# facebookresearch/dietgpu

Hardware: AMD Instinct MI355X
Metric: rans_encode_decode_GBps (higher is better)
Workload: dtype u8 (byte-wise rANS on the split exponent plane of 16-bit words); 1 GPU; 256x524288 bfloat16 N(0,1), float codec, probBits 10 (BASELINE config 3); per_gpu_batch_bytes=268435456, api=C ABI: dgpu_float_compress + dgpu_float_decompress

## Files before the change

dietgpu_amd/_lib.py:

```python
import ctypes as C
import os

from .build import LIB_PATH

_lib = None

u32, i32, sz, vp = C.c_uint32, C.c_int, C.c_size_t, C.c_void_p
_SIGS = {
    "dgpu_version": (C.c_char_p, []),
    "dgpu_abi_version": (u32, []),
    "dgpu_last_error": (C.c_char_p, []),
    "dgpu_last_checksum_mismatches": (C.c_uint32, [C.POINTER(C.c_int32), C.POINTER(C.c_uint32), C.POINTER(C.c_uint32), C.c_uint32]),
    "dgpu_ans_max_compressed_size": (u32, [u32]),
    "dgpu_float_max_compressed_size": (u32, [u32, u32]),
    "dgpu_ans_encode_temp_bytes": (sz, [u32, u32]),
    "dgpu_ans_decode_temp_bytes": (sz, [u32, u32, i32]),
    "dgpu_float_compress_temp_bytes": (sz, [u32, u32, u32]),
    "dgpu_float_decompress_temp_bytes": (sz, [u32, u32, u32, i32]),
    "dgpu_ans_encode_batch_stride": (i32, [vp, sz, vp, i32, i32, u32, vp, u32, u32, vp, vp, u32, vp, vp]),
    "dgpu_ans_encode_batch_pointer": (i32, [vp, sz, vp, i32, i32, u32, vp, vp, vp, vp, vp, vp]),
    "dgpu_ans_encode_batch_split_size": (i32, [vp, sz, vp, i32, i32, u32, vp, vp, vp, vp, u32, vp, vp]),
    "dgpu_ans_decode_batch_stride": (i32, [vp, sz, vp, i32, i32, u32, vp, u32, vp, u32, u32, vp, vp, vp, vp]),
    "dgpu_ans_decode_batch_pointer": (i32, [vp, sz, vp, i32, i32, u32, vp, vp, vp, vp, vp, vp, vp]),
    "dgpu_ans_decode_batch_split_size": (i32, [vp, sz, vp, i32, i32, u32, vp, vp, vp, vp, vp, vp, vp]),
# ... 25 lines not shown
    "dgpu_float_reduce_compress_scaled": (i32, [vp, sz, vp, u32, i32, i32, u32, u32, vp, vp, vp, C.c_float, vp, vp, vp, vp, vp, vp, vp]),
    "dgpu_float_reduce_norm_temp_bytes": (sz, [u32, u32, u32, i32]),
    "dgpu_float_decode_reduce_norm": (i32, [vp, sz, vp, u32, i32, i32, u32, u32, vp, vp, vp, C.c_float, vp, vp, vp, vp, vp, vp, vp]),
    "dgpu_float_reduce_compress_norm": (i32, [vp, sz, vp, u32, i32, i32, u32, u32, vp, vp, vp, C.c_float, vp, vp, vp, vp, vp, vp, vp, vp, vp]),
    "dgpu_float_compress_stride_capped": (i32, [vp, sz, vp, u32, i32, i32, u32, vp, u32, u32, vp, u32, u32, vp, vp]),
    "dgpu_float_decompress_stride_bounded": (i32, [vp, sz, vp, u32, i32, i32, u32, vp, u32, u32, vp, u32, u32, vp, vp, vp, vp]),
    "dgpu_float_get_compressed_info": (i32, [vp, sz, vp, u32, vp, vp, vp, vp]),
    "dgpu_float_get_compressed_info_device": (i32, [vp, u32, vp, vp, vp, vp]),
    "dgpu_ans_histogram_batch_stride": (i32, [u32, vp, u32, u32, vp, vp]),
    "dgpu_ans_calc_weights": (i32, [u32, i32, vp, u32, vp, vp, vp]),
    "dgpu_release_stream_state": (i32, [vp]),
    "dgpu_release_all_stream_state": (i32, []),
    "dgpu_debug_stream_state_count": (u32, []),
    "dgpu_debug_counters_nonzero": (C.c_int64, [vp]),
    "dgpu_prof_enable": (None, [i32]),
    "dgpu_prof_reset": (None, []),
    "dgpu_prof_summary": (i32, [C.c_char_p, sz]),
    "dgpu_debug_set_absent_workgroups": (None, [u32]),
    "dgpu_debug_set_encoder_dispatch": (None, [i32]),
    "dgpu_debug_set_decoder_order": (None, [i32]),
    "dgpu_debug_set_param_cache": (None, [i32]),
    "dgpu_debug_set_work_lists": (None, [i32]),
    "dgpu_debug_set_size_classes": (None, [i32]),
    "dgpu_set_histogram_load_policy": (None, [i32]),
    "dgpu_release_graph_state": (i32, []),
}

EXPORTED_SYMBOLS = tuple(_SIGS)


def lib():
    global _lib
    if _lib is None:
        if not os.path.exists(LIB_PATH):
            raise ImportError(
                f"{LIB_PATH} is missing: the HIP extension has not been built "
                "(run `python -m dietgpu_amd.build`). There is no CPU fallback."
            )
        L = C.CDLL(LIB_PATH)
        for name, (res, args) in _SIGS.items():
            if os.environ.get("DGPU_LIB") and not hasattr(L, name):
                continue
            fn = getattr(L, name)
            fn.restype = res
            fn.argtypes = args
        _lib = L
# ... 12 lines not shown
```

dietgpu_amd/build.py:

```python
import os
import subprocess

_HERE = os.path.dirname(os.path.abspath(__file__))
CSRC = os.path.join(_HERE, "csrc")
LIB_DIR = os.path.join(_HERE, "lib")
LIB_PATH = os.environ.get("DGPU_LIB") or os.path.join(LIB_DIR, "libdietgpu_amd.so")

_SOURCES = ["capi.hip"]


def _deps():
    names = sorted(f for f in os.listdir(CSRC) if f.endswith((".h", ".hip")))
    return [os.path.join(CSRC, f) for f in names] + [os.path.join(_HERE, "..", "include", "dietgpu_amd.h")]


def needs_build():
    if not os.path.exists(LIB_PATH):
        return True
    t = os.path.getmtime(LIB_PATH)
    return any(os.path.getmtime(d) > t for d in _deps())


def build(force=False, verbose=False):
    if not force and not needs_build():
        return LIB_PATH
    os.makedirs(LIB_DIR, exist_ok=True)
    cmd = ["hipcc", "--offload-arch=gfx950", "-O3", "-std=c++17", "-fPIC", "-shared",
           "-o", LIB_PATH] + [os.path.join(CSRC, s) for s in _SOURCES]
    if verbose:
        print(" ".join(cmd))
    subprocess.check_call(cmd)
    return LIB_PATH


TORCH_LIB_PATH = os.path.join(LIB_DIR, "libdietgpu_torch.so")


def build_torch_ops(force=False, verbose=False):
    src = os.path.join(CSRC, "torch_ops.cpp")
    if (not force and os.path.exists(TORCH_LIB_PATH)
            and os.path.getmtime(TORCH_LIB_PATH) >= max(os.path.getmtime(src), os.path.getmtime(LIB_PATH))):
        return TORCH_LIB_PATH
    import torch

    tl = os.path.dirname(torch.__file__)
    abi = int(torch._C._GLIBCXX_USE_CXX11_ABI)
    cmd = ["g++", "-O2", "-std=c++17", "-fPIC", "-shared", "-D__HIP_PLATFORM_AMD__", "-DUSE_ROCM",
           f"-D_GLIBCXX_USE_CXX11_ABI={abi}", f"-I{tl}/include", f"-I{tl}/include/torch/csrc/api/include",
           "-I/opt/rocm/include", src, "-o", TORCH_LIB_PATH, f"-L{LIB_DIR}", "-ldietgpu_amd", f"-L{tl}/lib",
           "-ltorch", "-ltorch_cpu", "-lc10", "-lc10_hip", "-ltorch_hip", "-Wl,-rpath,$ORIGIN"]
    if verbose:
        print(" ".join(cmd))
    subprocess.check_call(cmd)
    return TORCH_LIB_PATH
# ... 6 lines not shown
```

dietgpu_amd/csrc/capi.hip:

```cpp
#include "../../include/dietgpu_amd.h"

#include <hip/hip_runtime.h>

#include <algorithm>
#include <atomic>
#include <climits>
#include <cmath>
#include <cstdio>
#include <cstdlib>
#include <cstring>
#include <map>
#include <mutex>
#include <string>
#include <thread>
#include <vector>

#include "format.h"
#include "kernel_variants.h"
#include "work_plan.h"

using namespace dgpu;

namespace {

// ... 1071 lines not shown
  if (done) return rc;
  return encodeBatch(temp_dev, tempBytes, tempUsed, 0u, P, useChecksum, b, histogram_dev, outSize_dev, stream);
}

int floatCompressImpl(
    void* temp_dev, size_t tempBytes, size_t* tempUsed, uint32_t ft, int P, int useChecksum, Batch& b, uint32_t* outSize_dev,
    hipStream_t stream, bool cast = false, const RollingCounts& rolling = RollingCounts{}, bool feedback = false) {
  bool done;
  int rc = checkCall(P, b.n, ft, tempUsed,  nullptr, &done,
                     "tensor larger than 1717538816 words: the maximum compressed size of its exponent plane exceeds INT32_MAX (GpuANSEncode.cu:22)",
                     b.maxSize);
  if (done) return rc;
  const uint32_t source = feedback ? (ft | kCastSource | kFeedbackSource) : (cast ? (ft | kCastSource) : ft);
  return encodeBatch(temp_dev, tempBytes, tempUsed, source, P, useChecksum, b, nullptr, outSize_dev, stream, 0xffffffffu, rolling);
}

std::atomic<int> g_decOrder{envInt("DGPU_DEC_ORDER", -1)};
uint32_t decodeOrder(uint32_t B) {
  const int forced = g_decOrder.load();
  if (forced >= 0 && forced <= (int)kDecOrderXcd) return (uint32_t)forced;
  return B >= 64u ? kDecOrderXcd : kDecOrderElementMajor;
}

DecodeArgs decodeArgs(const Batch& b, const DeviceBatch& d, uint32_t ft, uint8_t* outSuccess_dev, uint32_t* outSize_dev) {
  DecodeArgs a;
  a.in = d.in;
  a.out = d.out;
  a.floatType = ft;
  a.outSuccess = outSuccess_dev;
  a.outSize = outSize_dev;
  a.inBytes = d.inBytes;
  a.uniformInBytes = b.uniformInBytes;
  a.numInBatch = b.n;
  return a;
}

int launchDecode(DecodeArgs d, const LaunchGroup& g, const uint32_t* work_dev, DecodeForm form, int P, hipStream_t stream) {
  const bool pairs = g.tileBlocks == kDecBlocksPerSingleTile;
  const uint32_t B = d.numInBatch;
  d.maxTiles = g.maxTiles;
  d.order = g.listed ? kDecOrderMap : decodeOrder(B);
  d.workMap = g.listed ? work_dev + (pairs ? g.elemsAt : g.tilesAt) : nullptr;
  d.numListed = g.numElems;
  const uint32_t tiles = g.listed ? std::max(g.numTiles, 1u) : (d.order == kDecOrderXcd ? roundUp(B, 8u) : B) * g.maxTiles;
  const uint32_t grid = pairs ? ((g.listed ? g.numElems : B) + 1u) / 2u : tiles;
  return launchVariant(decoderVariant(P, d.floatType, g.tileBlocks, form), dim3(grid), stream, d);
}

int decodeImpl(
    void* temp_dev, size_t tempBytes, size_t* tempUsed, uint32_t ft, int P, int useChecksum, Batch& b, uint8_t* outSuccess_dev,
    uint32_t* outSize_dev, hipStream_t stream, int32_t* errBatch) {
  g_mismatches.clear();
  bool done;
  int rc = checkCall(P, b.n, ft, tempUsed, errBatch, &done);
  if (done) return rc;
  const uint32_t B = b.n, maxCapacity = b.maxSize;
  StreamLease streamLease(stream);
  if (useChecksum && streamLease.capturing()) {
    return fail(DGPU_ERR_HIP, "HIP graph capture: checksum verification on decode copies to the host and synchronises the "
                              "stream; it cannot be captured into a HIP graph (decode with useChecksum = 0 under capture)");
  }

  TempArena arena(temp_dev, tempBytes, streamLease);
  DeviceBatch dev;
  std::vector<LaunchGroup> groups{decodeRectangle(divUp(maxCapacity, kBlockSize), true)};
  rc = resolveBatch(b, true, streamLease, &dev, [&] { planDecodeCall(planPolicy(), b.sizes, maxCapacity, true, &groups, &b.work); });
  if (rc) return rc;

  uint32_t* sizesForChecksum = outSize_dev;
// ... 392 lines not shown

uint32_t dgpu_last_checksum_mismatches(int32_t* batchIdx, uint32_t* expected, uint32_t* got, uint32_t cap) {
  const uint32_t n = (uint32_t)g_mismatches.size();
  for (uint32_t i = 0; i < n && i < cap; ++i) {
    if (batchIdx) batchIdx[i] = g_mismatches[i].batch;
    if (expected) expected[i] = g_mismatches[i].expected;
    if (got) got[i] = g_mismatches[i].got;
  }
  return n;
}

static std::atomic<uint32_t> g_absentModulo{0};
}
namespace {
uint32_t absentWorkgroupModulo() { return g_absentModulo.load(); }
}
extern "C" {
void dgpu_debug_set_absent_workgroups(uint32_t modulo) { g_absentModulo.store(modulo); }
void dgpu_debug_set_encoder_dispatch(int mode) { g_encDispatch.store(mode < 0 ? -1 : (mode != 0)); }
void dgpu_debug_set_decoder_order(int order) { g_decOrder.store(order); }
void dgpu_debug_set_param_cache(int on) { g_paramCacheEnabled.store(on != 0); }
void dgpu_debug_set_work_lists(int mode) { g_workLists.store(mode < 0 ? -1 : (mode ? 1 : 0)); }
void dgpu_debug_set_size_classes(int mode) { g_sizeClasses.store(mode < 0 ? -1 : (mode ? 1 : 0)); }
void dgpu_set_histogram_load_policy(int mode) { g_histLoadPolicy.store(mode < 0 ? -1 : (mode != 0)); }
int dgpu_release_graph_state(void) {
  const int n = paramCache().releaseGraphPins();
  return n + streamRegistry().release(nullptr, true, true);
}

int dgpu_release_stream_state(void* stream) { return streamRegistry().release((hipStream_t)stream, false); }
int dgpu_release_all_stream_state(void) { return streamRegistry().release(nullptr, true); }
uint32_t dgpu_debug_stream_state_count(void) { return (uint32_t)streamRegistry().size(); }
int64_t dgpu_debug_counters_nonzero(void* stream) {
  hipStreamCaptureStatus st = hipStreamCaptureStatusNone;
  if (hipStreamIsCapturing((hipStream_t)stream, &st) != hipSuccess || st != hipStreamCaptureStatusNone) {
    (void)hipGetLastError();
    return -1;
  }
  hipError_t e = hipSuccess;
  StreamState* s = streamRegistry().acquire((hipStream_t)stream, &e, false);
  if (!s) return -1;
  int64_t n = -1;
  std::vector<uint32_t> host(kCounterWordsArrive + kCounterWordsAcc + kCounterWordsSpill);
  if (s->counters && hipStreamSynchronize((hipStream_t)stream) == hipSuccess &&
      hipMemcpy(host.data(), s->counters, host.size() * sizeof(uint32_t), hipMemcpyDeviceToHost) == hipSuccess) {
    n = (int64_t)std::count_if(host.begin(), host.end(), [](uint32_t w) { return w != 0u; });
// ... 646 lines not shown
```

dietgpu_amd/csrc/kernel_variants.h:

```cpp
#pragma once

#include <hip/hip_runtime.h>

#include <map>
#include <mutex>
#include <type_traits>

#include "format.h"
#include "kernels_decode.h"
#include "kernels_encode.h"
#include "kernels_pairs.h"
#include "kernels_stats.h"

namespace dgpu {

template <typename... Args>
struct KernelVariant {
  void (*fn)(Args...);
  uint32_t threads;
  uint32_t ldsBytes;
  const char* name;
};
using EncodeVariant = KernelVariant<EncodeArgs>;
using DecodeVariant = KernelVariant<DecodeArgs>;
using HistogramVariant = KernelVariant<BatchView, uint32_t*, uint32_t, HistFuse>;
using StatsSingleVariant = KernelVariant<BatchView, NormalizeArgs, const uint32_t*, uint32_t>;

template <typename... Args>
uint32_t workgroupsPerCu(const KernelVariant<Args...>& v) {
  static std::mutex mu;
  static std::map<const void*, uint32_t> cache;
// ... 104 lines not shown
    return tiled(UintC<kBlocksPerTile>{}, yes, no);
  });
}

constexpr uint32_t sameType(uint32_t ft) { return ft; }
constexpr uint32_t floatsOnly(uint32_t ft) { return ft ? ft : kFloat32; }
constexpr uint32_t halvesOnly(uint32_t ft) { return ft == kFloat16 ? kFloat16 : kBFloat16; }

#define DGPU_DECODE_FORMS(X)                                                                                           \
  X(kAccum, k_ans_decode_accum, floatsOnly, decLdsBytes(P, T, TB))                                                     \
  X(kReduce, k_ans_decode_reduce, floatsOnly, decLdsBytes(P, T, TB))                                                   \
  X(kReduceStats, k_ans_decode_reduce_stats, halvesOnly, decReduceStatsLdsBytes(P, T, TB))                             \
  X(kReduceMixed, k_ans_decode_reduce_mixed, floatsOnly, decLdsBytes(P, T, TB))                                        \
  X(kReduceMixedStats, k_ans_decode_reduce_mixed_stats, halvesOnly, decReduceStatsLdsBytes(P, T, TB))                  \
  X(kReduceScaled, k_ans_decode_reduce_mixed_scaled, floatsOnly, decLdsBytes(P, T, TB))                                \
  X(kReduceScaledStats, k_ans_decode_reduce_mixed_stats_scaled, halvesOnly, decReduceStatsScaledLdsBytes(P, T, TB))    \
  X(kReduceNorm, k_ans_decode_reduce_mixed_norm, floatsOnly, decReduceNormLdsBytes(P, T, TB, false))                   \
  X(kReduceNormStats, k_ans_decode_reduce_mixed_stats_norm, halvesOnly, decReduceNormLdsBytes(P, T, TB, true))         \
  X(kWholeScaled, k_ans_decode_scaled, floatsOnly, decScaledLdsBytes(P, T, TB))                                        \
  X(kAccumScaled, k_ans_decode_accum_scaled, floatsOnly, decLdsBytes(P, T, TB))                                        \
  X(kUpdate, k_ans_decode_update, halvesOnly, decLdsBytes(P, T, TB))                                                   \
  X(kRanged, k_ans_decode_range, sameType, decLdsBytes(P, T, TB))

inline DecodeVariant decoderVariant(int P, uint32_t ft, uint32_t tileBlocks, DecodeForm form = DecodeForm::kWhole) {
  return withProbBitsAndFloatType(P, ft, [&](auto p, auto f) -> DecodeVariant {
    constexpr int kP = decltype(p)::value;
    constexpr uint32_t kFT = decltype(f)::value;
    auto smallOrFull = [&](auto tiled) -> DecodeVariant {
      return tileBlocks <= kDecBlocksPerSmallTile ? tiled(UintC<kDecBlocksPerSmallTile>{}) : tiled(UintC<kDecBlocksPerTile>{});
    };
#define DGPU_DECODE_FORM_CASE(formName, kernel, typeOf, ldsBytes)                \
  if (form == DecodeForm::formName) {                                            \
    return smallOrFull([](auto tb) -> DecodeVariant {                            \
      constexpr int P = kP;                                                      \
      constexpr uint32_t T = typeOf(kFT), TB = decltype(tb)::value;              \
      return {kernel<P, T, TB>, decThreads(TB), ldsBytes, #kernel};              \
    });                                                                          \
  }
    DGPU_DECODE_FORMS(DGPU_DECODE_FORM_CASE)
#undef DGPU_DECODE_FORM_CASE
    if (tileBlocks == kDecBlocksPerSingleTile) return {k_ans_decode_pair<kP, kFT>, 64u, decPairLdsBytes(kP, kFT), "k_ans_decode_pair"};
    auto tiled = [](auto tb) -> DecodeVariant {
      constexpr uint32_t kTB = decltype(tb)::value;
      return {k_ans_decode<kP, kFT, kTB>, decThreads(kTB), decLdsBytes(kP, kFT, kTB), "k_ans_decode"};
    };
    if (tileBlocks == kDecBlocksPerTinyTile) return tiled(UintC<kDecBlocksPerTinyTile>{});
    if (tileBlocks == kDecBlocksPerSmallTile) return tiled(UintC<kDecBlocksPerSmallTile>{});
    return tiled(UintC<kDecBlocksPerTile>{});
  });
}

inline HistogramVariant histogramVariant(uint32_t ft, bool smallBins, bool nonTemporal) {
  auto pick = [&](auto f) -> HistogramVariant {
    constexpr uint32_t kFT = decltype(f)::value;
    auto of = [](auto slots, auto nt) -> HistogramVariant {
      constexpr uint32_t kS = decltype(slots)::value;
      constexpr bool kNt = decltype(nt)::value;
      if constexpr (kFT == 0) {
        return {k_histogram<kS, kNt>, 256u, 0u, "k_histogram"};
      } else {
        return {k_float_histogram<kFT, kS, kNt>, 256u, 0u,
                encIsFeedback(kFT) ? "k_float_histogram_feedback" : (encIsCast(kFT) ? "k_float_histogram_cast" : "k_float_histogram")};
      }
    };
    constexpr UintC<kHistSlotsSmall> small{};
    constexpr UintC<kHistSlotsLarge> large{};
// ... 20 lines not shown
```

dietgpu_amd/csrc/kernels_decode.h:

```cpp
#pragma once
#include <type_traits>

#include "format.h"
#include "plan_constants.h"
#include "kernels_stats.h"

namespace dgpu {

__device__ __forceinline__ const uint8_t* locateAns(const uint8_t* archive, uint32_t ft, uint32_t* floatSize) {
  if (!ft) return archive;
  const FloatHeader fh = *(const FloatHeader*)archive;
  if (floatSize) *floatSize = fh.size;
  return archive + 16u + floatUncompDataSize(ft, fh.size);
}

struct DecodeArgs {
  BatchView in;
  BatchView out;
  uint32_t floatType;
  uint8_t* outSuccess;
  uint32_t* outSize;
  const uint32_t* inBytes;
  uint32_t numInBatch;
  uint32_t maxTiles;
// ... 592 lines not shown
struct DecodePreOf {
  uint4 words[4];
  GroupPre nc[2];
};
typedef DecodePreOf<uint2> DecodePre;
template <uint32_t FT, typename Sink>
__device__ __forceinline__ void decodePrefetch(DecodePreOf<typename Sink::GroupPre>& pre, const uint8_t* __restrict__ gwords, uint32_t numWords,
                                               const Sink& sink, uint32_t hl, bool wide) {
  const uint32_t paddedBytes = roundUp(numWords, kBlockAlignWords) * 2u;
#pragma unroll
  for (uint32_t k = 0; k < 4u; ++k) {
    const uint32_t off = (k * 32u + hl) * 16u;
    pre.words[k] = make_uint4(0, 0, 0, 0);
    if (off < paddedBytes) pre.words[k] = decLoad16(gwords + off);
  }
  pre.nc[0] = pre.nc[1] = typename Sink::GroupPre();
  if (wide) {
    pre.nc[0] = sink.prefetchGroup(kRowsPerBlock / 8u - 1u, hl);
    pre.nc[1] = sink.prefetchGroup(kRowsPerBlock / 8u - 2u, hl);
  }
}

template <int P, uint32_t FT, bool kFull, bool kWide = false, bool kIdleUpper = false, bool kCompact = false, bool kNoRing = false,
          bool kPre = false, bool kTail = false, typename Sink = RowSink<FT>>
__device__ __forceinline__ void decodeBlock(
    uint32_t xpose,
    uint32_t state,
    uint32_t n,
    uint32_t groups,
    const uint8_t* __restrict__ gwords,
    uint32_t numWords,
    uint32_t ringBase,
    const void* __restrict__ lutRaw,
    const Sink& sink,
    uint32_t hl,
    bool upper,
    const DecodePreOf<typename Sink::GroupPre>* pre = nullptr,
    uint32_t topRows = 0) {
  static_assert(!kPre || (kNoRing && kFull), "");
  static_assert(!kTail || (kFull && !kPre), "");
  constexpr uint32_t kMask = (1u << P) - 1u;
  const uint32_t laneMaskLt = (1u << hl) - 1u;
  auto lutAt = [&](uint32_t x) -> uint2 {
    if (kCompact) {
      const uint32_t e = ((const uint32_t*)lutRaw)[x];
      return make_uint2((e & 0xff000fffu), (e >> 12) & 0xfffu);
    }
// ... 57 lines not shown
  int upperSel = (upper && !kIdleUpper) ? 1 : 0;
  asm volatile("" : "+v"(upperSel));
  auto stepFull = [&]() -> uint32_t {
    const uint2 e = lutAt(state & kMask);
    state = __umul24(e.x, state >> P) + e.y;
    const bool read = state < kMinState;
    const uint64_t vote = __ballot(read);
    const uint32_t vLo = (uint32_t)vote, vHi = (uint32_t)(vote >> 32);
    const uint32_t sLoOld = sLo;
    sLo -= (uint32_t)__popc(vLo);
    sHi -= (uint32_t)__popc(vHi);
    uint32_t t = __builtin_amdgcn_mbcnt_hi(vHi, __builtin_amdgcn_mbcnt_lo(vLo, 0u));
    t = (uint32_t)(__mul24(upperSel, (int)(sHi - sLoOld)) + (int)t);
    asm volatile("" : "+v"(t));
    const uint32_t addr = kNoRing ? ((t + sLo) << 1) : ((((t + sLo) << 1) & (kRingBytes - 1u)) | ringBase);
    const uint32_t w = *(const LdsU16*)(uintptr_t)addr;
    state = read ? ((state << kEncodedBits) | w) : state;
    return e.x;
  };

  auto runGroups = [&](auto fullTag, const int gHi, const int gLo) {
    constexpr bool F = decltype(fullTag)::value;
    constexpr bool kJoinAtFlush = F && kWide;
    Pre preCur[kGroupRows], preNext[kGroupRows];
    GroupPre ncCur = GroupPre(), ncNext = GroupPre(), ncNext2 = GroupPre();
    if (kJoinAtFlush) {
      if (kPre) {
        ncCur = pre->nc[0];
        ncNext = pre->nc[1];
      } else {
        ncCur = sink.prefetchGroup((uint32_t)gHi, hl);
        ncNext = sink.prefetchGroup(gHi > gLo ? (uint32_t)(gHi - 1) : (uint32_t)gLo, hl);
      }
    }
#pragma unroll
    for (int j = 0; j < (int)kGroupRows; ++j) {
      const uint32_t row = (uint32_t)gHi * kGroupRows + j;
      preCur[j] = kJoinAtFlush ? (Pre)0 : ((F || row * 32u + hl < n) ? sink.prefetch(row) : (Pre)0);
    }

#pragma unroll 1
    for (int g = gHi; g >= gLo; --g) {
      const uint32_t gNext = g > gLo ? (uint32_t)(g - 1) : (uint32_t)gLo;
      if (kJoinAtFlush) {
        ncNext2 = sink.prefetchGroup(g > gLo + 1 ? (uint32_t)(g - 2) : (uint32_t)gLo, hl);
      } else {
// ... 39 lines not shown
      } else {
#pragma unroll
        for (int j = 0; j < (int)kGroupRows; ++j) preCur[j] = preNext[j];
      }
    }
  };

  if (kTail) {
    if (topRows != 0u) runGroups(std::false_type{}, (int)(groups + divUp(topRows, kGroupRows)) - 1, (int)groups);
    if (groups == 0u) return;
  }
  if (kFull) {
    sLo = __builtin_amdgcn_readlane(posw, 0);
    sHi = __builtin_amdgcn_readlane(posw, 32);
    if (kNoRing) {
      sLo += __builtin_amdgcn_readlane(ringBase, 0) >> 1;
      sHi += __builtin_amdgcn_readlane(ringBase, 32) >> 1;
    }
  }
  runGroups(std::integral_constant<bool, kFull>{}, (int)groups - 1, 0);
}

enum class DecodeForm { kWhole, kRanged, kAccum, kReduce, kReduceStats, kReduceMixed, kReduceMixedStats, kReduceScaled, kReduceScaledStats, kReduceNorm, kReduceNormStats, kWholeScaled, kAccumScaled, kUpdate };
template <int P, uint32_t FT, uint32_t kTileBlocks, DecodeForm kForm>
__device__ __forceinline__ void decodeTile(const DecodeArgs& a) {
  constexpr bool kRanged = kForm == DecodeForm::kRanged, kAccumScaled = kForm == DecodeForm::kAccumScaled;
  constexpr bool kUpdate = kForm == DecodeForm::kUpdate;
  constexpr bool kAccum = kForm == DecodeForm::kAccum || kAccumScaled || kUpdate;
  constexpr bool kScaledForm = kForm == DecodeForm::kWholeScaled || kAccumScaled || kUpdate;
  static_assert(kForm == DecodeForm::kWhole || kForm == DecodeForm::kRanged || kAccum || kScaledForm,
                "decode-reduce has a body of its own: decodeReduceTile");
  static_assert(!(kAccum || kScaledForm) || FT != 0u, "accumulating and scaled decode: float archives only");
  static_assert(!kUpdate || FT == kFloat16 || FT == kBFloat16, "decode-update: 16-bit float archives only");
  using Sink = std::conditional_t<kUpdate, UpdateSink<kUpdate ? FT : kBFloat16>,
                                  std::conditional_t<kAccum, AccumSink<FT ? FT : kFloat32, 0u, false, false, kAccumScaled>,
                                                     std::conditional_t<kScaledForm, ScaledSink<FT ? FT : kFloat32>, RowSink<FT>>>>;
  constexpr uint32_t kDecThreads = decThreads(kTileBlocks);
  static_assert(kTileBlocks * kRingBytes >= 2048u, "");
  extern __shared__ __attribute__((aligned(16))) uint8_t smem[];
  uint2* sLut = (uint2*)(smem + kTileBlocks * kRingBytes);
  constexpr uint32_t kXpose = decXposeBytes(P, FT, kTileBlocks);

  const uint32_t tid = threadIdx.x;
  const uint32_t lane = tid & 63u;
  const uint32_t wave = tid >> 6;
  const bool upper = lane >= 32u;
  const uint32_t hl = lane & 31u;
  const uint32_t hw = wave * 2u + (upper ? 1u : 0u);
// ... 241 lines not shown
        carry = dmax(carry, (uint32_t)__builtin_amdgcn_readlane((int)incl, 63));
      }
    } else
    for (uint32_t x = tid; x < (1u << P); x += kDecThreads) {
      uint32_t lo = 0, hi = kNumSymbols;
#pragma unroll
      for (int it = 0; it < 8; ++it) {
        const uint32_t mid = (lo + hi) >> 1;
        const bool le = sCdf[mid] <= x;
        lo = le ? mid : lo;
        hi = le ? hi : mid;
      }
      if (kCompact) ((uint32_t*)sLut)[x] = (sPdf[lo] & 0xfffu) | (((x - sCdf[lo]) & 0xfffu) << 12) | (lo << 24);
      else sLut[x] = make_uint2((sPdf[lo] & 0xfffu) | (lo << 24), (x - sCdf[lo]) & 0xfffu);
    }
  }

  __syncthreads();

  constexpr uint32_t kLutBytesHere = decLutBytes(P, kTileBlocks);
  const uint32_t xpose = ldsBase + kTileBlocks * kRingBytes + kLutBytesHere + hw * kXpose;
  const uint32_t ringLds = ldsBase + hw * kRingBytes;
#define DGPU_DECODE_FULL(WIDE, IDLE, NORING) \
  decodeBlock<P, FT, true, WIDE, IDLE, kCompact, NORING, NORING>(xpose, state, n, kRowsPerBlock / kGroupRows, gwords, numWords, ringLds, sLut, sink, hl, upper, &pre)
  if (fullPair) {
    if (wide) {
      if (noRing) DGPU_DECODE_FULL(true, false, true); else DGPU_DECODE_FULL(true, false, false);
    } else {
      if (noRing) DGPU_DECODE_FULL(false, false, true); else DGPU_DECODE_FULL(false, false, false);
    }
  } else if (fullSingle) {
    if (wide) {
      if (noRing) DGPU_DECODE_FULL(true, true, true); else DGPU_DECODE_FULL(true, true, false);
    } else {
      if (noRing) DGPU_DECODE_FULL(false, true, true); else DGPU_DECODE_FULL(false, true, false);
    }
#undef DGPU_DECODE_FULL
  } else {
    const uint32_t maxN = nFirst > nSecond ? nFirst : nSecond;
    const uint32_t maxRows = divUp(maxN, 32u);
    const uint32_t fullRows = (nSecond ? nSecond : nFirst) / 32u;
    const uint32_t groups = fullRows / kGroupRows;
    const uint32_t topRows = maxRows - groups * kGroupRows;
    const bool tailPair = nFirst == kBlockSize && nSecond != 0u, tailSingle = nFirst != 0u && nSecond == 0u;
    if ((tailPair || tailSingle) && groups != 0u) {
#define DGPU_DECODE_TAIL(WIDE, IDLE, NORING) \
  decodeBlock<P, FT, true, WIDE, IDLE, kCompact, NORING, false, true>(xpose, state, n, groups, gwords, numWords, ringLds, sLut, sink, hl, upper, nullptr, topRows)
      if (tailPair) {
        if (wide) {
          if (noRing) DGPU_DECODE_TAIL(true, false, true); else DGPU_DECODE_TAIL(true, false, false);
        } else {
          if (noRing) DGPU_DECODE_TAIL(false, false, true); else DGPU_DECODE_TAIL(false, false, false);
        }
      } else {
        if (wide) {
          if (noRing) DGPU_DECODE_TAIL(true, true, true); else DGPU_DECODE_TAIL(true, true, false);
        } else {
          if (noRing) DGPU_DECODE_TAIL(false, true, true); else DGPU_DECODE_TAIL(false, true, false);
        }
      }
#undef DGPU_DECODE_TAIL
    } else {
      decodeBlock<P, FT, false, false, false, kCompact>(xpose, state, n, divUp(maxRows, kGroupRows), gwords, numWords, ringLds, sLut, sink, hl, upper);
    }
  }
}

template <uint32_t FT, bool kRounded>
__device__ __forceinline__ uint32_t normWord(uint32_t o) {
  if constexpr (!kRounded) {
// ... 420 lines not shown
  }
  if constexpr (kStats) {
    __syncthreads();
    const uint32_t* bins = (const uint32_t*)(smem + kBinsAt);
    for (uint32_t c = tid; c < kNumSymbols; c += kDecThreads) {
      uint32_t sum = 0;
#pragma unroll
      for (uint32_t k = 0; k < kSlots / 4u; ++k) {
        const uint4 v = ((const uint4*)(bins + c * kSlots))[k];
        sum += v.x + v.y + v.z + v.w;
      }
      if (sum) __hip_atomic_fetch_add(a.stats + (size_t)b * kNumSymbols + c, sum, __ATOMIC_RELAXED, __HIP_MEMORY_SCOPE_AGENT);
    }
  }
  if constexpr (kNorm) reduceNormTile<FT, kStats, kDecThreads>((const ReduceNormTile*)(smem + kNormTileAt), smem);
}

template <int P, uint32_t FT, uint32_t kTileBlocks>
__global__ __launch_bounds__(decThreads(kTileBlocks)) void k_ans_decode(DecodeArgs a) {
  decodeTile<P, FT, kTileBlocks, DecodeForm::kWhole>(a);
}

template <int P, uint32_t FT, uint32_t kTileBlocks>
__global__ __launch_bounds__(decThreads(kTileBlocks)) void k_ans_decode_range(DecodeArgs a) {
  decodeTile<P, FT, kTileBlocks, DecodeForm::kRanged>(a);
}

template <int P, uint32_t FT, uint32_t kTileBlocks>
__global__ __launch_bounds__(decThreads(kTileBlocks)) void k_ans_decode_accum(DecodeArgs a) {
  decodeTile<P, FT, kTileBlocks, DecodeForm::kAccum>(a);
}

__host__ __device__ constexpr uint32_t decScaledLdsBytes(int P, uint32_t ft, uint32_t tileBlocks) { return decLdsBytes(P, ft, tileBlocks); }
template <int P, uint32_t FT, uint32_t kTileBlocks>
__global__ __launch_bounds__(decThreads(kTileBlocks)) void k_ans_decode_scaled(DecodeArgs a) {
  static_assert(FT != 0u, "scaled decode: float archives only");
  decodeTile<P, FT, kTileBlocks, DecodeForm::kWholeScaled>(a);
}

template <int P, uint32_t FT, uint32_t kTileBlocks>
__global__ __launch_bounds__(decThreads(kTileBlocks)) void k_ans_decode_accum_scaled(DecodeArgs a) {
  static_assert(FT != 0u, "accumulating decode: float archives only");
  decodeTile<P, FT, kTileBlocks, DecodeForm::kAccumScaled>(a);
}

template <int P, uint32_t FT, uint32_t kTileBlocks>
// ... 40 lines not shown
}

__host__ __device__ constexpr uint32_t decReduceNormLdsBytes(int P, uint32_t ft, uint32_t tileBlocks, bool stats) {
  return (stats ? decReduceStatsScaledLdsBytes(P, ft, tileBlocks) : decLdsBytes(P, ft, tileBlocks)) + (uint32_t)sizeof(ReduceNormTile);
}
template <int P, uint32_t FT, uint32_t kTileBlocks>
__global__ __launch_bounds__(decThreads(kTileBlocks)) void k_ans_decode_reduce_mixed_norm(DecodeArgs a) {
  decodeReduceTile<P, FT, kTileBlocks, false, true, true, true>(a);
}
template <int P, uint32_t FT, uint32_t kTileBlocks>
__global__ __launch_bounds__(decThreads(kTileBlocks)) void k_ans_decode_reduce_mixed_stats_norm(DecodeArgs a) {
  static_assert(FT == kFloat16 || FT == kBFloat16, "the archive types of a cast");
  decodeReduceTile<P, FT, kTileBlocks, true, true, true, true>(a);
}

struct ReduceNormFinishArgs {
  const double* partials;
  uint32_t numInBatch, maxTiles;
  double* outSumSq;
  uint32_t* outNonFinite;
};
constexpr uint32_t kNormFinishThreads = 256;
__host__ __device__ constexpr size_t reduceNormPartialBytes(size_t numInBatch, size_t maxTiles) { return numInBatch * maxTiles * 12u; }
__global__ __launch_bounds__(kNormFinishThreads) void k_reduce_norm_finish(ReduceNormFinishArgs a) {
  const uint32_t lane = threadIdx.x & 63u;
  const uint32_t b = blockIdx.x * (kNormFinishThreads / 64u) + (threadIdx.x >> 6);
  if (b >= a.numInBatch) return;
  const double* partSq = a.partials + (size_t)b * a.maxTiles;
  const uint32_t* partBad = (const uint32_t*)(a.partials + (size_t)a.numInBatch * a.maxTiles) + (size_t)b * a.maxTiles;
  double sq = 0.0;
  uint32_t bad = 0;
  for (uint32_t t = lane; t < a.maxTiles; t += 64u) {
    sq += partSq[t];
    bad += partBad[t];
  }
#pragma unroll
  for (int d = 32; d >= 1; d >>= 1) {
    sq += __shfl_xor(sq, d, 64);
    bad += __shfl_xor(bad, d, 64);
  }
  if (lane == 0u) {
    if (a.outSumSq) a.outSumSq[b] = sq;
    if (a.outNonFinite) a.outNonFinite[b] = bad;
  }
}

}
// ... 1 lines not shown
```

dietgpu_amd/csrc/kernels_stats.h:

```cpp
#pragma once

#include "format.h"

namespace dgpu {

__device__ __forceinline__ uint32_t waveReduceSum(uint32_t v) {
#pragma unroll
  for (int m = 32; m >= 1; m >>= 1) v += __shfl_xor(v, m, 64);
  return v;
}
__device__ __forceinline__ uint32_t waveReduceXor(uint32_t v) {
#pragma unroll
  for (int m = 32; m >= 1; m >>= 1) v ^= __shfl_xor(v, m, 64);
  return v;
}
__device__ __forceinline__ uint32_t waveInclusiveScan(uint32_t v, uint32_t lane) {
#pragma unroll
  for (int d = 1; d < 64; d <<= 1) {
    uint32_t t = __shfl_up(v, d, 64);
    if (lane >= (uint32_t)d) v += t;
  }
  return v;
}

// ... 248 lines not shown
    cdf = waveBase + incl - pdf;

  }

  if (a.countsOut) a.countsOut[(size_t)b * kNumSymbols + tid] = 0u;
  if (a.encTable) a.encTable[b * kNumSymbols + tid] = encTableEntry(pdf, cdf, P);
  if (a.refTable) {
    uint32_t magic = 0, shift = 0;
    if (pdf > 0) {
      shift = 32u - (uint32_t)__clz((int)(pdf - 1u));
      const uint64_t one = 1;
      uint64_t magic64 = ((one << 32) * ((one << shift) - (uint64_t)pdf)) / (uint64_t)pdf + 1;
      magic = (uint32_t)magic64;
    }
    a.refTable[b * kNumSymbols + tid] = make_uint4(pdf, cdf, magic, shift);
  }

  if (ans) {
    ((uint16_t*)(ans + sizeof(AnsHeader)))[tid] = (uint16_t)pdf;
    if (tid == 0) normWriteHeader(a, b, total, ans);
  }
}

__global__ __launch_bounds__(256) void k_normalize(NormalizeArgs a) {
  __shared__ __attribute__((aligned(16))) uint32_t sScratch[kNormScratchWords];
  normalizeElement<false>(a, blockIdx.x, sScratch);
}

struct HistFuse {
  uint32_t* arrive;
  uint32_t* acc;
  NormalizeArgs norm;
  const uint32_t* workMap;
  uint32_t partBytes;
  BatchView residual;
};

struct HistWork {
  uint32_t b, part, parts, slot;
};
__device__ __forceinline__ HistWork histWorkOf(const HistFuse& f, const BatchView& in, uint32_t wordBytes) {
  HistWork w;
  if (f.workMap) {
    const uint32_t m = f.workMap[blockIdx.x];
    w.b = m >> 16;
    w.part = m & 0xffffu;
    const uint64_t bytes = (uint64_t)in.size(w.b) * wordBytes;
// ... 159 lines not shown
    const uint4 v0 = streamLoad<kNt>(&pv[i]), v1 = streamLoad<kNt>(&pv[i + 256u]), v2 = streamLoad<kNt>(&pv[i + 512u]), v3 = streamLoad<kNt>(&pv[i + 768u]);
    histAdd4<S>(myBins, v0.x); histAdd4<S>(myBins, v0.y); histAdd4<S>(myBins, v0.z); histAdd4<S>(myBins, v0.w);
    histAdd4<S>(myBins, v1.x); histAdd4<S>(myBins, v1.y); histAdd4<S>(myBins, v1.z); histAdd4<S>(myBins, v1.w);
    histAdd4<S>(myBins, v2.x); histAdd4<S>(myBins, v2.y); histAdd4<S>(myBins, v2.z); histAdd4<S>(myBins, v2.w);
    histAdd4<S>(myBins, v3.x); histAdd4<S>(myBins, v3.y); histAdd4<S>(myBins, v3.z); histAdd4<S>(myBins, v3.w);
  }
  for (; i < vEnd; i += 256u) {
    const uint4 v = streamLoad<kNt>(&pv[i]);
    histAdd4<S>(myBins, v.x);
    histAdd4<S>(myBins, v.y);
    histAdd4<S>(myBins, v.z);
    histAdd4<S>(myBins, v.w);
  }

  if (w.part == 0) {
    uint32_t t = numVec * 16u + tid;
    if (t < remaining) histAdd<S>(myBins, p[head + t]);
  }
  __syncthreads();

  histStore(hist, partial, fuse, w, tid, histFold<S>(bins, tid));
}

__global__ __launch_bounds__(256) void k_checksum(
    BatchView in, const uint32_t* __restrict__ sizesOverride, const uint8_t* __restrict__ onlyIf,
    uint32_t* __restrict__ out) {
  __shared__ uint32_t partial[4];
  const uint32_t tid = threadIdx.x;
  const uint32_t b = blockIdx.y;
  if (onlyIf && !onlyIf[b]) return;
  const uint8_t* p = in.ptr(b);
  uint32_t size = sizesOverride ? sizesOverride[b] : in.size(b);

  uint32_t head = (uint32_t)((16u - ((uintptr_t)p & 15u)) & 15u);
  head = head < size ? head : size;
  const uint32_t remaining = size - head;
  const uint32_t numVec = remaining / 16u;
  const uint4* pv = (const uint4*)(p + head);

  uint32_t c = 0;
  if (blockIdx.x == 0 && tid < head) c ^= p[tid];
  for (uint32_t i = blockIdx.x * 256u + tid; i < numVec; i += gridDim.x * 256u) {
    uint4 v = pv[i];
    c ^= v.x ^ v.y ^ v.z ^ v.w;
  }
  if (blockIdx.x == 0) {
    uint32_t i = numVec * 16u + tid;
    if (i < remaining) c ^= p[head + i];
  }
  c = (c ^ (c >> 8) ^ (c >> 16) ^ (c >> 24)) & 0xffu;
  c = waveReduceXor(c);
  if ((tid & 63u) == 0) partial[tid >> 6] = c;
  __syncthreads();
  if (tid == 0) {
    c = partial[0] ^ partial[1] ^ partial[2] ^ partial[3];
    if (c) atomicXor(&out[b], c);
  }
}

__global__ void k_ans_info(
    BatchView in, uint32_t numInBatch, uint32_t* outSizes, uint32_t* outChecksum) {
  uint32_t b = blockIdx.x * blockDim.x + threadIdx.x;
  if (b >= numInBatch) return;
  const AnsHeader* h = (const AnsHeader*)in.ptr(b);
  bool ok = h->magicAndVersion == ((kAnsMagic << 16) | kAnsVersion);
  if (outSizes) outSizes[b] = ok ? h->totalUncompressedWords : 0u;
  if (outChecksum) outChecksum[b] = ok ? h->checksum : 0u;
}

__global__ void k_float_info(
    BatchView in, uint32_t numInBatch, uint32_t* outSizes, uint32_t* outTypes,
    uint32_t* outChecksum) {
  uint32_t b = blockIdx.x * blockDim.x + threadIdx.x;
  if (b >= numInBatch) return;
  const FloatHeader* h = (const FloatHeader*)in.ptr(b);
  bool ok = h->magicAndVersion == ((kFloatMagic << 16) | kFloatVersion);
  if (outSizes) outSizes[b] = ok ? h->size : 0u;
  if (outTypes) outTypes[b] = ok ? (h->options & 0xfu) : 0u;
  if (outChecksum) outChecksum[b] = ok ? h->checksum : 0u;
}

}
```

include/dietgpu_amd.h:

```cpp
#ifndef DIETGPU_AMD_H
#define DIETGPU_AMD_H

#include <stddef.h>
#include <stdint.h>

#ifdef __cplusplus
extern "C" {
#endif

#define DGPU_OK 0
#define DGPU_ERR_INVALID_ARGUMENT 1
#define DGPU_ERR_HIP 2
#define DGPU_ERR_CHECKSUM_MISMATCH 3

#define DGPU_FLOAT_UNDEFINED 0u
#define DGPU_FLOAT16 1u
#define DGPU_BFLOAT16 2u
#define DGPU_FLOAT32 3u

#define DGPU_ANS_REQUIRED_ALIGNMENT 4
#define DGPU_ANS_DEFAULT_PROB_BITS 10

const char* dgpu_version(void);
#define DGPU_ABI_VERSION 8u
// ... 296 lines not shown
    const uint32_t* histogram_dev,
    uint32_t* table_dev,
    void* stream);

int dgpu_release_stream_state(void* stream);
int dgpu_release_all_stream_state(void);
uint32_t dgpu_debug_stream_state_count(void);
int64_t dgpu_debug_counters_nonzero(void* stream);

void dgpu_prof_enable(int on);
void dgpu_prof_reset(void);
int dgpu_prof_summary(char* buf, size_t cap);

void dgpu_debug_set_absent_workgroups(uint32_t modulo);

void dgpu_debug_set_encoder_dispatch(int mode);

void dgpu_debug_set_decoder_order(int order);

void dgpu_debug_set_work_lists(int mode);

void dgpu_debug_set_size_classes(int mode);

void dgpu_debug_set_param_cache(int on);

void dgpu_set_histogram_load_policy(int mode);

int dgpu_release_graph_state(void);

#ifdef __cplusplus
}
#endif
#endif
```

Baseline: 2237 GB/s.

## Add named-buffer rotating prefetch group loop to 16-bit tiled ANS decoder

Adds a decode kernel variant whose wide full-group loop keeps three named GroupPre prefetch buffers (two for tails), rotating them in an unrolled-by-depth loop instead of copying preCur/preNext arrays. The aim is to keep prefetches in fixed registers and avoid the buffer shuffling between groups. It is on by default for float16 and bfloat16, and an env var and debug setter can turn it off. The new kernel is compiled in a separate translation unit with a parallel split build, and some shared kernels are marked static there to avoid duplicate symbols.

Result: no change. 2245 GB/s (median of 6 runs) (+0.4%).

```diff
diff --git a/dietgpu_amd/_lib.py b/dietgpu_amd/_lib.py
--- a/dietgpu_amd/_lib.py
+++ b/dietgpu_amd/_lib.py
@@ -71,6 +71,7 @@
     "dgpu_debug_set_param_cache": (None, [i32]),
     "dgpu_debug_set_work_lists": (None, [i32]),
     "dgpu_debug_set_size_classes": (None, [i32]),
+    "dgpu_debug_set_decode_group_loop": (None, [i32]),
     "dgpu_set_histogram_load_policy": (None, [i32]),
     "dgpu_release_graph_state": (i32, []),
 }
diff --git a/dietgpu_amd/build.py b/dietgpu_amd/build.py
--- a/dietgpu_amd/build.py
+++ b/dietgpu_amd/build.py
@@ -6,7 +6,7 @@
 LIB_DIR = os.path.join(_HERE, "lib")
 LIB_PATH = os.environ.get("DGPU_LIB") or os.path.join(LIB_DIR, "libdietgpu_amd.so")
 
-_SOURCES = ["capi.hip"]
+_SOURCES = ["capi.hip", "decode_nbuf.hip"]
 
 
 def _deps():
@@ -25,11 +25,23 @@
     if not force and not needs_build():
         return LIB_PATH
     os.makedirs(LIB_DIR, exist_ok=True)
-    cmd = ["hipcc", "--offload-arch=gfx950", "-O3", "-std=c++17", "-fPIC", "-shared",
-           "-o", LIB_PATH] + [os.path.join(CSRC, s) for s in _SOURCES]
+    flags = ["hipcc", "--offload-arch=gfx950", "-O3", "-std=c++17", "-fPIC"]
+    objects, running = [], []
+    for s in _SOURCES:
+        objects.append(os.path.join(LIB_DIR, os.path.splitext(s)[0] + ".o"))
+        cmd = flags + ["-DDGPU_SPLIT_BUILD", "-c", "-o", objects[-1], os.path.join(CSRC, s)]
+        if verbose:
+            print(" ".join(cmd), flush=True)
+        running.append((cmd, subprocess.Popen(cmd)))
+    failed = [cmd for cmd, p in running if p.wait() != 0]
+    if failed:
+        raise subprocess.CalledProcessError(1, failed[0])
+    cmd = flags + ["-shared", "-o", LIB_PATH] + objects
     if verbose:
-        print(" ".join(cmd))
+        print(" ".join(cmd), flush=True)
     subprocess.check_call(cmd)
+    for o in objects:
+        os.remove(o)
     return LIB_PATH
 
 
diff --git a/dietgpu_amd/csrc/capi.hip b/dietgpu_amd/csrc/capi.hip
--- a/dietgpu_amd/csrc/capi.hip
+++ b/dietgpu_amd/csrc/capi.hip
@@ -1117,6 +1117,8 @@
   return B >= 64u ? kDecOrderXcd : kDecOrderElementMajor;
 }
 
+std::atomic<int> g_decGroupLoop{envInt("DGPU_DEC_GROUP_LOOP", -1)};
+
 DecodeArgs decodeArgs(const Batch& b, const DeviceBatch& d, uint32_t ft, uint8_t* outSuccess_dev, uint32_t* outSize_dev) {
   DecodeArgs a;
   a.in = d.in;
@@ -1139,7 +1141,7 @@
   d.numListed = g.numElems;
   const uint32_t tiles = g.listed ? std::max(g.numTiles, 1u) : (d.order == kDecOrderXcd ? roundUp(B, 8u) : B) * g.maxTiles;
   const uint32_t grid = pairs ? ((g.listed ? g.numElems : B) + 1u) / 2u : tiles;
-  return launchVariant(decoderVariant(P, d.floatType, g.tileBlocks, form), dim3(grid), stream, d);
+  return launchVariant(decoderVariant(P, d.floatType, g.tileBlocks, form, g_decGroupLoop.load() != 0), dim3(grid), stream, d);
 }
 
 int decodeImpl(
@@ -1578,6 +1580,7 @@
 void dgpu_debug_set_param_cache(int on) { g_paramCacheEnabled.store(on != 0); }
 void dgpu_debug_set_work_lists(int mode) { g_workLists.store(mode < 0 ? -1 : (mode ? 1 : 0)); }
 void dgpu_debug_set_size_classes(int mode) { g_sizeClasses.store(mode < 0 ? -1 : (mode ? 1 : 0)); }
+void dgpu_debug_set_decode_group_loop(int mode) { g_decGroupLoop.store(mode < 0 ? -1 : (mode ? 1 : 0)); }
 void dgpu_set_histogram_load_policy(int mode) { g_histLoadPolicy.store(mode < 0 ? -1 : (mode != 0)); }
 int dgpu_release_graph_state(void) {
   const int n = paramCache().releaseGraphPins();
diff --git a/dietgpu_amd/csrc/decode_nbuf.hip b/dietgpu_amd/csrc/decode_nbuf.hip
--- /dev/null
+++ b/dietgpu_amd/csrc/decode_nbuf.hip
@@ -0,0 +1,7 @@
+#include <hip/hip_runtime.h>
+
+#include <cstdint>
+
+#define DGPU_NBUF_TU
+#define DGPU_PLAIN_KERNEL static
+#include "decode_nbuf_kernels.h"
diff --git a/dietgpu_amd/csrc/decode_nbuf_kernels.h b/dietgpu_amd/csrc/decode_nbuf_kernels.h
--- /dev/null
+++ b/dietgpu_amd/csrc/decode_nbuf_kernels.h
@@ -0,0 +1,31 @@
+#pragma once
+
+#include "kernels_decode.h"
+
+namespace dgpu {
+
+using DecodeKernel = void (*)(DecodeArgs);
+
+#if defined(DGPU_SPLIT_BUILD) && !defined(DGPU_NBUF_TU)
+DecodeKernel namedBufferDecodeKernel(int P, uint32_t ft, uint32_t tileBlocks);
+#else
+#ifndef DGPU_NBUF_TU
+inline
+#endif
+DecodeKernel namedBufferDecodeKernel(int P, uint32_t ft, uint32_t tileBlocks) {
+#define DGPU_NBUF_TILES(P, T)                                                          \
+  return tileBlocks == kDecBlocksPerTinyTile    ? k_ans_decode_nbuf<P, T, kDecBlocksPerTinyTile>   \
+         : tileBlocks == kDecBlocksPerSmallTile ? k_ans_decode_nbuf<P, T, kDecBlocksPerSmallTile>  \
+                                                : k_ans_decode_nbuf<P, T, kDecBlocksPerTile>
+#define DGPU_NBUF_TYPES(P)                            \
+  if (ft == kFloat16) { DGPU_NBUF_TILES(P, kFloat16); } \
+  DGPU_NBUF_TILES(P, kBFloat16)
+  if (P == 9) { DGPU_NBUF_TYPES(9); }
+  if (P == 10) { DGPU_NBUF_TYPES(10); }
+  DGPU_NBUF_TYPES(11);
+#undef DGPU_NBUF_TYPES
+#undef DGPU_NBUF_TILES
+}
+#endif
+
+}
diff --git a/dietgpu_amd/csrc/kernel_variants.h b/dietgpu_amd/csrc/kernel_variants.h
--- a/dietgpu_amd/csrc/kernel_variants.h
+++ b/dietgpu_amd/csrc/kernel_variants.h
@@ -7,6 +7,7 @@
 #include <type_traits>
 
 #include "format.h"
+#include "decode_nbuf_kernels.h"
 #include "kernels_decode.h"
 #include "kernels_encode.h"
 #include "kernels_pairs.h"
@@ -157,7 +158,7 @@
   X(kUpdate, k_ans_decode_update, halvesOnly, decLdsBytes(P, T, TB))                                                   \
   X(kRanged, k_ans_decode_range, sameType, decLdsBytes(P, T, TB))
 
-inline DecodeVariant decoderVariant(int P, uint32_t ft, uint32_t tileBlocks, DecodeForm form = DecodeForm::kWhole) {
+inline DecodeVariant decoderVariant(int P, uint32_t ft, uint32_t tileBlocks, DecodeForm form = DecodeForm::kWhole, bool namedBufferLoop = true) {
   return withProbBitsAndFloatType(P, ft, [&](auto p, auto f) -> DecodeVariant {
     constexpr int kP = decltype(p)::value;
     constexpr uint32_t kFT = decltype(f)::value;
@@ -175,8 +176,11 @@
     DGPU_DECODE_FORMS(DGPU_DECODE_FORM_CASE)
 #undef DGPU_DECODE_FORM_CASE
     if (tileBlocks == kDecBlocksPerSingleTile) return {k_ans_decode_pair<kP, kFT>, 64u, decPairLdsBytes(kP, kFT), "k_ans_decode_pair"};
-    auto tiled = [](auto tb) -> DecodeVariant {
-      constexpr uint32_t kTB = decltype(tb)::value;
+    auto tiled = [&](auto tb) -> DecodeVariant {
+      constexpr uint32_t kTB = decltype(tb)::value;
+      if constexpr (kFT == kFloat16 || kFT == kBFloat16) {
+        if (namedBufferLoop) return {namedBufferDecodeKernel(kP, kFT, kTB), decThreads(kTB), decLdsBytes(kP, kFT, kTB), "k_ans_decode"};
+      }
       return {k_ans_decode<kP, kFT, kTB>, decThreads(kTB), decLdsBytes(kP, kFT, kTB), "k_ans_decode"};
     };
     if (tileBlocks == kDecBlocksPerTinyTile) return tiled(UintC<kDecBlocksPerTinyTile>{});
diff --git a/dietgpu_amd/csrc/kernels_decode.h b/dietgpu_amd/csrc/kernels_decode.h
--- a/dietgpu_amd/csrc/kernels_decode.h
+++ b/dietgpu_amd/csrc/kernels_decode.h
@@ -638,7 +638,7 @@
 }
 
 template <int P, uint32_t FT, bool kFull, bool kWide = false, bool kIdleUpper = false, bool kCompact = false, bool kNoRing = false,
-          bool kPre = false, bool kTail = false, typename Sink = RowSink<FT>>
+          bool kPre = false, bool kTail = false, typename Sink = RowSink<FT>, bool kNamedBufferLoop = false>
 __device__ __forceinline__ void decodeBlock(
     uint32_t xpose,
     uint32_t state,
@@ -742,6 +742,52 @@
   auto runGroups = [&](auto fullTag, const int gHi, const int gLo) {
     constexpr bool F = decltype(fullTag)::value;
     constexpr bool kJoinAtFlush = F && kWide;
+    if constexpr (kNamedBufferLoop && kJoinAtFlush) {
+      constexpr int kDepth = kTail ? 2 : 3;
+      GroupPre a, b, c = GroupPre();
+      if (kPre) {
+        a = pre->nc[0];
+        b = pre->nc[1];
+      } else {
+        a = sink.prefetchGroup((uint32_t)gHi, hl);
+        b = sink.prefetchGroup(gHi > gLo ? (uint32_t)(gHi - 1) : (uint32_t)gLo, hl);
+      }
+      if constexpr (kDepth == 3) c = sink.prefetchGroup(gHi > gLo + 1 ? (uint32_t)(gHi - 2) : (uint32_t)gLo, hl);
+      auto groupBody = [&](int g, GroupPre& buf) {
+        if (!kNoRing) {
+          posw = upper ? sHi : sLo;
+          if (pendingChunk >= 0) {
+            *(LdsU4*)(uintptr_t)(ringBase | (((uint32_t)pendingChunk & 3u) * 512u + hl * 16u)) = u32x4{pending.x, pending.y, pending.z, pending.w};
+            pendingChunk = -1;
+          }
+          if (lowChunk > 0 && (uint32_t)lowChunk * kRingChunkWords + 512u > posw) {
+            --lowChunk;
+            const uint32_t off = (uint32_t)lowChunk * 512u + hl * 16u;
+            pending = (off < paddedBytes) ? decLoad16(gwords + off) : make_uint4(0, 0, 0, 0);
+            pendingChunk = lowChunk;
+          }
+        }
+#pragma unroll
+        for (int j = (int)kGroupRows - 1; j >= 0; --j) {
+          const uint32_t e0 = stepFull();
+          if (!kIdleUpper || !upper) sink.stageRow(xpose, (uint32_t)j, hl, e0);
+        }
+        if (!kIdleUpper || !upper) sink.flushGroup(xpose, (uint32_t)g, hl, buf);
+        buf = sink.prefetchGroup(g >= gLo + kDepth ? (uint32_t)(g - kDepth) : (uint32_t)gLo, hl);
+      };
+      int g = gHi;
+#pragma unroll 1
+      for (; g - (kDepth - 1) >= gLo; g -= kDepth) {
+        groupBody(g, a);
+        groupBody(g - 1, b);
+        if constexpr (kDepth == 3) groupBody(g - 2, c);
+      }
+      if (g >= gLo) groupBody(g, a);
+      if constexpr (kDepth == 3) {
+        if (g - 1 >= gLo) groupBody(g - 1, b);
+      }
+      return;
+    }
     Pre preCur[kGroupRows], preNext[kGroupRows];
     GroupPre ncCur = GroupPre(), ncNext = GroupPre(), ncNext2 = GroupPre();
     if (kJoinAtFlush) {
@@ -827,8 +873,10 @@
 }
 
 enum class DecodeForm { kWhole, kRanged, kAccum, kReduce, kReduceStats, kReduceMixed, kReduceMixedStats, kReduceScaled, kReduceScaledStats, kReduceNorm, kReduceNormStats, kWholeScaled, kAccumScaled, kUpdate };
-template <int P, uint32_t FT, uint32_t kTileBlocks, DecodeForm kForm>
+template <int P, uint32_t FT, uint32_t kTileBlocks, DecodeForm kForm, bool kNamedBufferLoop = false>
 __device__ __forceinline__ void decodeTile(const DecodeArgs& a) {
+  static_assert(!kNamedBufferLoop || (kForm == DecodeForm::kWhole && (FT == kFloat16 || FT == kBFloat16)),
+                "the named-buffer group loop: the whole decode of the 16-bit types only");
   constexpr bool kRanged = kForm == DecodeForm::kRanged, kAccumScaled = kForm == DecodeForm::kAccumScaled;
   constexpr bool kUpdate = kForm == DecodeForm::kUpdate;
   constexpr bool kAccum = kForm == DecodeForm::kAccum || kAccumScaled || kUpdate;
@@ -1116,7 +1164,7 @@
   const uint32_t xpose = ldsBase + kTileBlocks * kRingBytes + kLutBytesHere + hw * kXpose;
   const uint32_t ringLds = ldsBase + hw * kRingBytes;
 #define DGPU_DECODE_FULL(WIDE, IDLE, NORING) \
-  decodeBlock<P, FT, true, WIDE, IDLE, kCompact, NORING, NORING>(xpose, state, n, kRowsPerBlock / kGroupRows, gwords, numWords, ringLds, sLut, sink, hl, upper, &pre)
+  decodeBlock<P, FT, true, WIDE, IDLE, kCompact, NORING, NORING, false, Sink, kNamedBufferLoop>(xpose, state, n, kRowsPerBlock / kGroupRows, gwords, numWords, ringLds, sLut, sink, hl, upper, &pre)
   if (fullPair) {
     if (wide) {
       if (noRing) DGPU_DECODE_FULL(true, false, true); else DGPU_DECODE_FULL(true, false, false);
@@ -1139,7 +1187,7 @@
     const bool tailPair = nFirst == kBlockSize && nSecond != 0u, tailSingle = nFirst != 0u && nSecond == 0u;
     if ((tailPair || tailSingle) && groups != 0u) {
 #define DGPU_DECODE_TAIL(WIDE, IDLE, NORING) \
-  decodeBlock<P, FT, true, WIDE, IDLE, kCompact, NORING, false, true>(xpose, state, n, groups, gwords, numWords, ringLds, sLut, sink, hl, upper, nullptr, topRows)
+  decodeBlock<P, FT, true, WIDE, IDLE, kCompact, NORING, false, true, Sink, kNamedBufferLoop>(xpose, state, n, groups, gwords, numWords, ringLds, sLut, sink, hl, upper, nullptr, topRows)
       if (tailPair) {
         if (wide) {
           if (noRing) DGPU_DECODE_TAIL(true, false, true); else DGPU_DECODE_TAIL(true, false, false);
@@ -1606,6 +1654,11 @@
 }
 
 template <int P, uint32_t FT, uint32_t kTileBlocks>
+__global__ __launch_bounds__(decThreads(kTileBlocks)) void k_ans_decode_nbuf(DecodeArgs a) {
+  decodeTile<P, FT, kTileBlocks, DecodeForm::kWhole, true>(a);
+}
+
+template <int P, uint32_t FT, uint32_t kTileBlocks>
 __global__ __launch_bounds__(decThreads(kTileBlocks)) void k_ans_decode_range(DecodeArgs a) {
   decodeTile<P, FT, kTileBlocks, DecodeForm::kRanged>(a);
 }
@@ -1692,7 +1745,7 @@
 };
 constexpr uint32_t kNormFinishThreads = 256;
 __host__ __device__ constexpr size_t reduceNormPartialBytes(size_t numInBatch, size_t maxTiles) { return numInBatch * maxTiles * 12u; }
-__global__ __launch_bounds__(kNormFinishThreads) void k_reduce_norm_finish(ReduceNormFinishArgs a) {
+DGPU_PLAIN_KERNEL __global__ __launch_bounds__(kNormFinishThreads) void k_reduce_norm_finish(ReduceNormFinishArgs a) {
   const uint32_t lane = threadIdx.x & 63u;
   const uint32_t b = blockIdx.x * (kNormFinishThreads / 64u) + (threadIdx.x >> 6);
   if (b >= a.numInBatch) return;
diff --git a/dietgpu_amd/csrc/kernels_stats.h b/dietgpu_amd/csrc/kernels_stats.h
--- a/dietgpu_amd/csrc/kernels_stats.h
+++ b/dietgpu_amd/csrc/kernels_stats.h
@@ -1,4 +1,8 @@
 #pragma once
+
+#ifndef DGPU_PLAIN_KERNEL
+#define DGPU_PLAIN_KERNEL
+#endif
 
 #include "format.h"
 
@@ -294,7 +298,7 @@
   }
 }
 
-__global__ __launch_bounds__(256) void k_normalize(NormalizeArgs a) {
+DGPU_PLAIN_KERNEL __global__ __launch_bounds__(256) void k_normalize(NormalizeArgs a) {
   __shared__ __attribute__((aligned(16))) uint32_t sScratch[kNormScratchWords];
   normalizeElement<false>(a, blockIdx.x, sScratch);
 }
@@ -500,7 +504,7 @@
   histStore(hist, partial, fuse, w, tid, histFold<S>(bins, tid));
 }
 
-__global__ __launch_bounds__(256) void k_checksum(
+DGPU_PLAIN_KERNEL __global__ __launch_bounds__(256) void k_checksum(
     BatchView in, const uint32_t* __restrict__ sizesOverride, const uint8_t* __restrict__ onlyIf,
     uint32_t* __restrict__ out) {
   __shared__ uint32_t partial[4];
@@ -536,7 +540,7 @@
   }
 }
 
-__global__ void k_ans_info(
+DGPU_PLAIN_KERNEL __global__ void k_ans_info(
     BatchView in, uint32_t numInBatch, uint32_t* outSizes, uint32_t* outChecksum) {
   uint32_t b = blockIdx.x * blockDim.x + threadIdx.x;
   if (b >= numInBatch) return;
@@ -546,7 +550,7 @@
   if (outChecksum) outChecksum[b] = ok ? h->checksum : 0u;
 }
 
-__global__ void k_float_info(
+DGPU_PLAIN_KERNEL __global__ void k_float_info(
     BatchView in, uint32_t numInBatch, uint32_t* outSizes, uint32_t* outTypes,
     uint32_t* outChecksum) {
   uint32_t b = blockIdx.x * blockDim.x + threadIdx.x;
diff --git a/include/dietgpu_amd.h b/include/dietgpu_amd.h
--- a/include/dietgpu_amd.h
+++ b/include/dietgpu_amd.h
@@ -342,6 +342,8 @@
 
 void dgpu_debug_set_size_classes(int mode);
 
+void dgpu_debug_set_decode_group_loop(int mode);
+
 void dgpu_debug_set_param_cache(int on);
 
 void dgpu_set_histogram_load_policy(int mode);
```
